# TxCorpi0x/concrete

Measured on AMD Instinct MI355X. Metric: PBS/sec (whole node) at N=1024 batch=4096; achieved HBM GB/s, higher is better.
Workload: dtype u64

## Files before the change

concrete_amd/csrc/pbs.hip:

```cpp
#include <type_traits>

#include "common.hpp"
#include "fft512.hpp"
#include "kernel_util.hpp"
#include "pbs.hpp"
#include "pbs1024_plan.hpp"
#include "pbs_hex.hpp"

namespace chip {

constexpr uint64_t MAGIC_ALL = RND_MAGIC_BITS + (RND_MAGIC_BITS << 22) + (RND_MAGIC_BITS << 43);
constexpr int limb_shift(int li) { return li * 21 + (li > 0 ? 1 : 0); }

#ifndef FWD_LAST_VIA_WINDOW
#define FWD_LAST_VIA_WINDOW 1
#endif
#ifndef FWD_TW2_EARLY
#define FWD_TW2_EARLY 1
#endif
#ifndef DIAG_NOMAC
#define DIAG_NOMAC 0
#endif

#ifndef FWD_XBATCH
#define FWD_XBATCH 2
#endif
#ifndef PAIR_FLAGS
#define PAIR_FLAGS 1
#endif

__device__ __forceinline__ void pair_signal(uint32_t* flags, int w, uint32_t& cnt) {
  asm volatile("" ::: "memory");
  ++cnt;
#if !defined(DIAG_NOXBAR)
  __hip_atomic_store(&flags[w], cnt, __ATOMIC_RELAXED, __HIP_MEMORY_SCOPE_WORKGROUP);
#endif
}
__device__ __forceinline__ void pair_wait(uint32_t* flags, int w, uint32_t cnt, const SyncGuard& guard) {
#if defined(DIAG_NOXBAR)
  (void)flags, (void)w, (void)cnt, (void)guard;
#else
  spin_until_ge(&flags[w ^ 1], cnt, guard);
#endif
  asm volatile("" ::: "memory");
}
__device__ __forceinline__ void xchg_barrier(uint32_t* flags, int w, uint32_t& cnt, const SyncGuard& guard) {
#if defined(DIAG_NOXBAR)
  (void)flags, (void)w, (void)cnt, (void)guard;
  asm volatile("s_waitcnt lgkmcnt(0)" ::: "memory");
#elif PAIR_FLAGS
  asm volatile("s_waitcnt lgkmcnt(0)" ::: "memory");
  ++cnt;
  __hip_atomic_store(&flags[w], cnt, __ATOMIC_RELAXED, __HIP_MEMORY_SCOPE_WORKGROUP);
  spin_until_ge(&flags[w ^ 1], cnt, guard);
#else
  (void)flags, (void)w, (void)cnt, (void)guard;
  pair_barrier();
#endif
}

template <int P, int L, bool RESID, bool STAMPS>
__global__ void __launch_bounds__(P * 128, 2)
pbs1024_pair_kernel(uint64_t* __restrict__ out, const uint64_t* __restrict__ out_idx,
                    const uint64_t* __restrict__ luts, const uint64_t* __restrict__ lut_idx,
                    const uint64_t* __restrict__ in, const uint64_t* __restrict__ in_idx,
                    const cplx* __restrict__ fbsk, uint32_t n, uint32_t base_log, uint32_t num_samples,
                    unsigned long long* __restrict__ resid_out, SyncGuard guard) {
  constexpr int K = 1, K1 = 2, N = 1024, LOG2_2N = 11, LIMBS = 3, RQ = K1 * L;
  constexpr int PER_I = K1 * LIMBS * RQ * 512;
  static_assert(XCH_SLOTS <= (int)PBS1024_XCH_SLOTS, "transpose scratch");
  static_assert(FFT512_TABLE_ENTRIES * sizeof(cplx) == PBS1024_TABLE_BYTES, "table bytes");
  constexpr int NW = 2 * P;
  constexpr int GROUP = L * 512;
  constexpr int NGRP = K1 * K1 * LIMBS;
  constexpr int GLDS = GROUP / 64 / NW;
  static_assert(GROUP % (64 * NW) == 0, "group split");

  extern __shared__ __attribute__((aligned(16))) char smem[];
  cplx* tbl = reinterpret_cast<cplx*>(smem);
  cplx* xch_all = tbl + FFT512_TABLE_ENTRIES;
  cplx* ring = xch_all + NW * PBS1024_XCH_SLOTS;
  uint32_t* pflags = reinterpret_cast<uint32_t*>(ring + 3 * GROUP);

  const int w = __builtin_amdgcn_readfirstlane(threadIdx.x >> 6);
  const int h = w & 1;
  const uint64_t hsign = (uint64_t)h << 63;
  const int lane = threadIdx.x & 63;
  const uint32_t s = blockIdx.x * P + (w >> 1);
  const bool active = s < num_samples;
  cplx* xch = xch_all + w * PBS1024_XCH_SLOTS;
  uint64_t* xch64 = reinterpret_cast<uint64_t*>(xch);
  cplx* mybox = xch;
  const cplx* partnerbox = xch_all + (w ^ 1) * PBS1024_XCH_SLOTS;
  cplx* partnermail = xch_all + (w ^ 1) * PBS1024_XCH_SLOTS;

  static_assert(NGRP % 3 == 0, "ring slot of a group must not depend on the step");
  const cplx* key_w = fbsk + (uint64_t)w * GLDS * 64;
  cplx* ring_w = ring + w * GLDS * 64;
  const uint32_t lane_b = (uint32_t)lane * (uint32_t)sizeof(cplx);
  auto issue_group = [&](const cplx* key_step, int r) __attribute__((always_inline)) {
    const char* src = reinterpret_cast<const char*>(key_step + r * GROUP);
    cplx* dst = ring_w + (r % 3) * GROUP;
#pragma unroll
    for (int j = 0; j < GLDS; ++j)
    {
      const cplx* gp = reinterpret_cast<const cplx*>(src + j * 1024 + lane_b);
      const uint32_t m0 = (uint32_t)(uintptr_t)(lds_ptr_t)(dst + j * 64);
#pragma clang diagnostic push
#pragma clang diagnostic ignored "-Winline-asm"
      asm volatile("s_mov_b32 m0, %1\n\tglobal_load_lds_dwordx4 %0, off" : : "v"(gp), "s"(m0) : "m0", "memory");
#pragma clang diagnostic pop
    }
  };
  if (n > 0) {
    issue_group(key_w, 0);
    issue_group(key_w, 1);
  }

  build_fft512_tables(tbl, threadIdx.x, P * 128);
  if (lane == 0) pflags[w] = 0u;
  uint32_t pcnt = 0;
  __syncthreads();
  const Fft512Tables T = fft512_tables_at(tbl);

  const uint64_t* lwe = in + (active ? (in_idx ? in_idx[s] : s) : 0) * (uint64_t)(n + 1);
  const uint64_t* lut = luts + (active && lut_idx ? lut_idx[s] : 0ull) * (uint64_t)(K1 * N);

  uint64_t B[16];
  {
    const uint32_t bt = active ? modswitch(lwe[n], LOG2_2N) : 0u;
#pragma unroll
    for (int m = 0; m < 16; ++m) {
      const uint32_t src = (uint32_t)(lane + 64 * m + bt) & (2 * N - 1);
      const uint64_t v = active ? lut[h * N + (src & (N - 1))] : 0ull;
      B[m] = src < N ? 0ull - v : v;
    }
  }

  const int nrep = 64 - L * (int)base_log;
  const int logB = (int)base_log;
  const int32_t neg_base = -(1 << logB);
  const uint32_t half_m1 = (1u << (logB - 1)) - 1u;
  double max_resid = 0.0;
  uint64_t acc_t[NSTAMP] = {};
  uint64_t t_begin = 0, tp = 0;
  if constexpr (STAMPS) t_begin = stamp();

  cplx tw3[4];
  fwd_p3_tw(tw3, T, lane);

  uint64_t a_next = active ? lwe[0] : 0ull;
  for (uint32_t i = 0; i < n; ++i) {
    const cplx* key_step = key_w + (uint64_t)i * PER_I;
    const uint64_t ai = a_next;
    if (i + 1 < n) a_next = active ? lwe[i + 1] : 0ull;

    const uint32_t at = modswitch(ai, LOG2_2N);
    if constexpr (STAMPS) {
      tp = stamp();
      acc_t[7] += ai != 0ull && at != 0u;
    }

    uint32_t st[16];
    {
#pragma unroll
      for (int m = 0; m < 16; ++m) xch64[lane + 64 * m] = B[m];
      wave_lds_fence();
      const uint32_t o0 = ((uint32_t)(lane - (int)at) << 3) + 8u * N;
      const uint32_t khi = 1u << (nrep - 33);
      uint64_t rv[16];
#pragma unroll
      for (int m = 0; m < 16; ++m)
        rv[m] = *reinterpret_cast<const uint64_t*>(reinterpret_cast<const char*>(xch64) + ((o0 + 512u * m) & 8191u));
      __builtin_amdgcn_sched_barrier(0);
#pragma unroll
      for (int m = 0; m < 16; ++m) {
        const uint32_t o = o0 + 512u * m;
        const uint32_t s32 = (uint32_t)((int32_t)(o << 18) >> 31);
        const uint64_t rvs = rv[m] ^ (((uint64_t)s32 << 32) | s32);
        const uint64_t x = B[m] + rvs + (uint64_t)(s32 & 1u);
        st[m] = ((uint32_t)(x >> 32) + khi) >> (nrep - 32);
      }
      wave_lds_fence();
    }
    if constexpr (STAMPS) {
      uint64_t t = stamp();
      acc_t[0] += t - tp;
      tp = t;
    }

    cplx Xo[L][4], Xp[L][4];
    constexpr int XB = FWD_XBATCH;
#pragma unroll
    for (int q0 = 0; q0 < L; q0 += XB) {
      const int nq = (q0 + XB <= L) ? XB : L - q0;
      cplx out[XB][4];
      {
#pragma unroll
        for (int t = 0; t < XB; ++t) {
          if (t < nq) {
            cplx v[8];
            int32_t d[16];
#pragma unroll
            for (int m = 0; m < 16; ++m)
              d[m] = decomp_level32(st[m], (uint32_t)((q0 + t) * logB), logB, half_m1, neg_base, q0 + t + 1 < L);
#pragma unroll
            for (int m = 0; m < 8; ++m) v[m] = {(double)d[m], (double)d[m + 8]};
            cplx tw2[4];
            fwd_p2_tw(tw2, T, lane >> 3);
            if (FWD_TW2_EARLY) __builtin_amdgcn_sched_barrier(0);
            fft512_fwd_tw(v, xch, lane, tw2, tw3, hsign, [&]() __attribute__((always_inline)) {
              if (q0 > 0 && t == 0) pair_wait(pflags, w, pcnt, guard);
            });
#pragma unroll
            for (int j = 0; j < 4; ++j) {
              Xo[q0 + t][j] = v[j];
              out[t][j] = v[4 + j];
            }
          }
        }
#pragma unroll
        for (int t = 0; t < XB; ++t)
          if (t < nq)
#pragma unroll
            for (int j = 0; j < 4; ++j) mybox[(t * 4 + j) * 64 + lane] = out[t][j];
      }
      const bool last_batch = q0 + XB >= L;
      if (!last_batch || !FWD_LAST_VIA_WINDOW) {
        xchg_barrier(pflags, w, pcnt, guard);
#pragma unroll
        for (int t = 0; t < XB; ++t)
          if (t < nq)
#pragma unroll
            for (int j = 0; j < 4; ++j) Xp[q0 + t][j] = partnerbox[(t * 4 + j) * 64 + lane];
      }
#pragma unroll
      for (int t = 0; t < XB; ++t)
        if (t < nq)
#pragma unroll
          for (int j = 0; j < 4; ++j) pin(Xo[q0 + t][j]);
      if (q0 + XB < L) pair_signal(pflags, w, pcnt);
    }
    if constexpr (STAMPS) {
      uint64_t t = stamp();
      acc_t[1] += t - tp;
      tp = t;
    }

    auto recombine = [&](const cplx (&v)[8], auto LIc) __attribute__((always_inline)) {
      constexpr int lr = decltype(LIc)::value;
#pragma unroll
      for (int m = 0; m < 8; ++m) {
        const double tr = RND_MAGIC - v[m].re, ti = RND_MAGIC - v[m].im;
        if constexpr (RESID) {
          max_resid = fmax(max_resid, fabs(v[m].re - (RND_MAGIC - tr)));
          max_resid = fmax(max_resid, fabs(v[m].im - (RND_MAGIC - ti)));
        }
        if constexpr (lr == 0) {
          B[m] += (uint64_t)__double_as_longlong(tr) - MAGIC_ALL;
          B[m + 8] += (uint64_t)__double_as_longlong(ti) - MAGIC_ALL;
        } else {
          B[m] += (uint64_t)__double_as_longlong(tr) << limb_shift(lr);
          B[m + 8] += (uint64_t)__double_as_longlong(ti) << limb_shift(lr);
        }
      }
    };
    static_for<0, LIMBS>([&](auto LI) __attribute__((always_inline)) {
      constexpr int li = decltype(LI)::value;
      cplx Ymine[4];
#pragma unroll
      for (int co = 0; co < K1; ++co) {
        cplx Y[4];
        if constexpr (DIAG_NOMAC) {
#pragma unroll
          for (int j = 0; j < 4; ++j) Y[j] = {0.0, 0.0};
        }
#pragma unroll
        for (int ro = 0; ro < K1; ++ro) {
          const int r = (li * K1 + co) * K1 + ro;
          const bool last_step = i + 1 >= n;
          if constexpr (STAMPS) {
            uint64_t t = stamp();
            acc_t[2] += t - tp;
            tp = t;
          }
          if (r + 1 < NGRP || !last_step) wait_vmcnt<GLDS>();
          else wait_vmcnt<0>();
          if constexpr (STAMPS) {
            uint64_t t = stamp();
            acc_t[8] += t - tp;
            tp = t;
          }
#ifndef DIAG_NOBAR
          pair_barrier();
#endif
          if constexpr (STAMPS) {
            uint64_t t = stamp();
            acc_t[5] += t - tp;
            tp = t;
          }
#ifndef DIAG_NODMA
          if (r + 2 < NGRP) issue_group(key_step, r + 2);
          else if (!last_step) issue_group(key_step + PER_I, r + 2 - NGRP);
#endif
          if constexpr (FWD_LAST_VIA_WINDOW && li == 0) {
            if (co == 0 && ro == 0) {
              constexpr int QL = (L - 1) / FWD_XBATCH * FWD_XBATCH;
#pragma unroll
              for (int q = QL; q < L; ++q)
#pragma unroll
                for (int j = 0; j < 4; ++j) Xp[q][j] = partnerbox[((q - QL) * 4 + j) * 64 + lane];
            }
          }
          const cplx* G = ring + (r % 3) * GROUP + (4 * h) * 64 + lane;
          cplx gv[L][4];
#pragma unroll
          for (int q = 0; q < L; ++q)
#pragma unroll
            for (int j = 0; j < 4; ++j) gv[q][j] = G[(q * 8 + j) * 64];
#pragma unroll
          for (int q = 0; q < (DIAG_NOMAC ? 0 : L); ++q) {
#pragma unroll
            for (int j = 0; j < 4; ++j) {
              const cplx x = ro == 0 ? Xo[q][j] : Xp[q][j];
              if (ro == 0 && q == 0) {
                Y[j].re = __builtin_fma(x.re, gv[q][j].re, -x.im * gv[q][j].im);
                Y[j].im = __builtin_fma(x.re, gv[q][j].im, x.im * gv[q][j].re);
              } else {
                Y[j].re = __builtin_fma(x.re, gv[q][j].re, __builtin_fma(-x.im, gv[q][j].im, Y[j].re));
                Y[j].im = __builtin_fma(x.re, gv[q][j].im, __builtin_fma(x.im, gv[q][j].re, Y[j].im));
              }
            }
          }
#pragma unroll
          for (int j = 0; j < 4; ++j) pin(Y[j]);
        }
        if (co == 0) {
#pragma unroll
          for (int j = 0; j < 4; ++j) Ymine[j] = Y[j];
        } else {
#pragma unroll
          for (int j = 0; j < 4; ++j) partnermail[j * 64 + lane] = Y[j];
        }
      }
      if constexpr (STAMPS) {
        uint64_t t = stamp();
        acc_t[2] += t - tp;
        tp = t;
      }
      xchg_barrier(pflags, w, pcnt, guard);
      cplx vp[8];
#pragma unroll
      for (int j = 0; j < 4; ++j) {
        vp[j] = Ymine[j];
        vp[4 + j] = mybox[j * 64 + lane];
      }
      if constexpr (STAMPS) {
        uint64_t t = stamp();
        acc_t[3] += t - tp;
        tp = t;
      }
      cplx gi2[4];
      inv_p2_stage_tw(gi2, T, lane & 7);
      fft512_inv_tw(vp, xch, T, lane, gi2, hsign);
      recombine(vp, LI);
#pragma unroll
      for (int m = 0; m < 16; ++m) pin(B[m]);
      if constexpr (RESID) pin(max_resid);
      if constexpr (STAMPS) {
        uint64_t t = stamp();
        acc_t[4] += t - tp;
        tp = t;
      }
    });
  }

  if constexpr (STAMPS) {
    acc_t[6] = stamp() - t_begin;
    if (lane == 0 && resid_out) {
      unsigned long long* dst = resid_out + ((uint64_t)blockIdx.x * NW + w) * NSTAMP;
      for (int q = 0; q < NSTAMP; ++q) dst[q] = acc_t[q];
    }
  }

  uint64_t* o = out + (active ? (out_idx ? out_idx[s] : s) : 0) * (uint64_t)(K * N + 1);
  if (!active) {
  } else if (h == 0) {
#pragma unroll
    for (int m = 0; m < 16; ++m) xch64[lane + 64 * m] = B[m];
    wave_lds_fence();
#pragma unroll
    for (int m = 0; m < 16; ++m) {
      const int j = lane + 64 * m;
      const uint64_t v = xch64[(N - j) & (N - 1)];
      o[j] = j == 0 ? 0ull - v : v;
    }
  } else if (lane == 0) {
    o[K * N] = 0ull - B[0];
  }

  if constexpr (RESID && !STAMPS) {
    for (int off = 32; off > 0; off >>= 1) max_resid = fmax(max_resid, __shfl_xor(max_resid, off));
    if (lane == 0 && active && resid_out) atomicMax(resid_out, (unsigned long long)__double_as_longlong(max_resid));
  }
}

template <int P, int L, bool RESID, bool STAMPS>
static int launch_pair_t(const PbsArgs& a) {
  const size_t lds = pbs1024_pair_lds_bytes(L, P);
  if (!pbs1024_exact(1, L, a.base_log)) {
    set_error("pbs: N=1024 l=%d logB=%u is outside the exact range", L, a.base_log);
    return -2;
  }
  auto kern = pbs1024_pair_kernel<P, L, RESID, STAMPS>;
  CHIP_CHECK(hipFuncSetAttribute((const void*)kern, hipFuncAttributeMaxDynamicSharedMemorySize, (int)lds));
  const uint32_t blocks = (a.num_samples + P - 1) / P;
  hipLaunchKernelGGL(kern, dim3(blocks), dim3(P * 128), lds, a.stream, a.out, a.out_idx, a.luts, a.lut_idx,
                     a.in, a.in_idx, reinterpret_cast<const cplx*>(a.fbsk), a.n, a.base_log, a.num_samples, a.resid,
                     a.guard);
  hipError_t e = hipGetLastError();
  if (e != hipSuccess) {
    set_error("pbs launch failed: %s", hipGetErrorString(e));
    return -1;
  }
  return 0;
}

static uint32_t device_cus() {
  static uint32_t cus[64] = {};
  int dev = 0;
  CHIP_CHECK(hipGetDevice(&dev));
  if (dev < 0 || dev >= 64) return 256;
  if (!cus[dev]) {
    int n = 0;
    CHIP_CHECK(hipDeviceGetAttribute(&n, hipDeviceAttributeMultiprocessorCount, dev));
    cus[dev] = n > 0 ? (uint32_t)n : 256u;
  }
  return cus[dev];
}

template <int P, int L>
static int launch_pair_p(const PbsArgs& a) {
  static const bool stamps = getenv("CONCRETE_HIP_PBS_STAMPS") && atoi(getenv("CONCRETE_HIP_PBS_STAMPS"));
  if (stamps) return launch_pair_t<P, L, true, true>(a);
  return a.resid ? launch_pair_t<P, L, true, false>(a) : launch_pair_t<P, L, false, false>(a);
}

static PbsArgs pbs_args_range(const PbsArgs& a, uint32_t start, uint32_t count) {
  PbsArgs r = a;
  r.num_samples = count;
  if (a.in_idx) r.in_idx = a.in_idx + start;
  else r.in = a.in + (uint64_t)start * (a.n + 1);
  if (a.out_idx) r.out_idx = a.out_idx + start;
  else r.out = a.out + (uint64_t)start * (a.k * a.N + 1);
  if (a.lut_idx) r.lut_idx = a.lut_idx + start;
  return r;
}

template <int L>
static int launch_pair(const PbsArgs& a) {
  if (a.num_samples == 0) return 0;
  const char* fe = getenv("CONCRETE_HIP_PBS_PAIRS");
  const int forced = fe ? atoi(fe) : 0;
  const uint32_t cus = device_cus();
  const int P = forced == 1 || forced == 2 || forced == 4 ? forced
                : a.num_samples <= cus ? 1 : a.num_samples <= 2 * cus ? 2 : 4;
  if (L == 3) {
    const char* he = getenv("CONCRETE_HIP_PBS_HEX");
    const int hx = he ? atoi(he) : -1;
    if (hx == 1 || hx == 2) return pbs1024_hex_launch(a, hx);
    if (hx != 0 && !fe && !getenv("CONCRETE_HIP_PBS_QUAD") && !getenv("CONCRETE_HIP_PBS_STAMPS")) {
      const Pbs1024Plan plan = plan_pbs1024(a.num_samples, cus);
      uint32_t start = 0;
      int rc = 0;
      if (plan.pair) {
        rc = launch_pair_p<4, L>(pbs_args_range(a, start, plan.pair));
        start += plan.pair;
      }
      if (rc == 0 && plan.hex2) {
        rc = pbs1024_hex_launch(pbs_args_range(a, start, plan.hex2), 2);
        start += plan.hex2;
      }
      if (rc == 0 && plan.hex1) rc = pbs1024_hex_launch(pbs_args_range(a, start, plan.hex1), 1);
      return rc;
    }
  }
  if (L == 3 && P <= 2 && !getenv("CONCRETE_HIP_PBS_STAMPS")) {
    const char* qe = getenv("CONCRETE_HIP_PBS_QUAD");
    const int q = qe ? atoi(qe) : -1;
    if (q == 1 || q == 2) return pbs1024_quad_launch(a, q);
    if (q != 0 && P == 1) return pbs1024_quad_launch(a, 1);
  }
  if (P == 1) return launch_pair_p<1, L>(a);
  if (P == 2) return launch_pair_p<2, L>(a);
  return launch_pair_p<4, L>(a);
}

int pbs_launch(const PbsArgs& a) {
  const KeyKind kind = key_format(a.k, a.N, a.level).kind;
  if (kind == KeyKind::GENERIC) return pbs_generic_launch(a);
  if (kind == KeyKind::N2048) return pbs2048_launch(a);
  if (kind == KeyKind::K2N1024) return pbs1024k2_launch(a);
  if (kind == KeyKind::SMALL) return pbs_small_launch(a);
  if (kind == KeyKind::N1024 && a.limbs == 3) {
    switch (a.level) {
      case 1: return launch_pair<1>(a);
      case 2: return launch_pair<2>(a);
      case 3: return launch_pair<3>(a);
      default: break;
    }
  }
  set_error("unsupported PBS parameters: N=%u k=%u level=%u limbs=%u", a.N, a.k, a.level, a.limbs);
  return -2;
}

}
```

Baseline: 100,800.

## Add frequency-slot pair PBS kernel with mailbox exchange and make it default

Adds a new N=1024, l=3 PBS kernel in which each of eight waves owns one frequency slot. Forward FFT outputs are exchanged through per-wave LDS mailboxes guarded by counter-based signalling, and key loads are software-prefetched PF steps ahead, including across iterations. The goal is to spread the external-product MAC work across waves and overlap the FFT, key loads and exchange. This costs more LDS, atomic counter spins and extra barriers, and with SLOT_DEFAULT the new kernel replaces the pair path in the planned launch.

After: 107,300 (median of 6 runs). 6.4% higher.

```diff
diff --git a/concrete_amd/csrc/pbs.hip b/concrete_amd/csrc/pbs.hip
--- a/concrete_amd/csrc/pbs.hip
+++ b/concrete_amd/csrc/pbs.hip
@@ -405,6 +405,339 @@
   }
 }
 
+#ifndef SLOT_PF
+#define SLOT_PF 6
+#endif
+#ifndef SLOT_FWD_PAIR
+#define SLOT_FWD_PAIR 1
+#endif
+#ifndef SLOT_Y_EARLY
+#define SLOT_Y_EARLY 1
+#endif
+#ifndef SLOT_QMAJOR
+#define SLOT_QMAJOR 1
+#endif
+#ifndef SLOT_DEFAULT
+#define SLOT_DEFAULT 1
+#endif
+constexpr int SLOT_MBOX = 512;
+constexpr size_t pbs1024_pair_slot_lds_bytes() {
+  return PBS1024_TABLE_BYTES + 2 * (size_t)PBS_PAIRS * (PBS1024_XCH_SLOTS + SLOT_MBOX) * 16 + 16;
+}
+
+__device__ __forceinline__ void slot_signal(uint32_t* ctr, int lane, uint32_t& cnt) {
+  asm volatile("" ::: "memory");
+  ++cnt;
+  if (lane == 0) __hip_atomic_fetch_add(ctr, 1u, __ATOMIC_RELAXED, __HIP_MEMORY_SCOPE_WORKGROUP);
+}
+
+template <bool RESID, bool STAMPS>
+__global__ void __launch_bounds__(PBS_PAIRS * 128, 2)
+pbs1024_pair_slot_kernel(uint64_t* __restrict__ out, const uint64_t* __restrict__ out_idx,
+                         const uint64_t* __restrict__ luts, const uint64_t* __restrict__ lut_idx,
+                         const uint64_t* __restrict__ in, const uint64_t* __restrict__ in_idx,
+                         const cplx* __restrict__ fbsk, uint32_t n, uint32_t base_log, uint32_t num_samples,
+                         unsigned long long* __restrict__ resid_out, SyncGuard guard) {
+  constexpr int K = 1, K1 = 2, N = 1024, LOG2_2N = 11, LIMBS = 3, L = 3, P = PBS_PAIRS, NW = 2 * P;
+  constexpr int GROUP = L * 512;
+  constexpr int PER_I = K1 * K1 * LIMBS * GROUP;
+  constexpr int NKEY = LIMBS * K1 * K1 * L;
+  constexpr int PF = SLOT_PF;
+  constexpr int XS = (int)PBS1024_XCH_SLOTS, MB = SLOT_MBOX;
+  static_assert(NW == 8, "one frequency slot per wave");
+  static_assert(NKEY % PF == 0, "a key value's register must not depend on the step");
+  static_assert(XCH_SLOTS <= XS, "transpose scratch");
+
+  extern __shared__ __attribute__((aligned(16))) char smem[];
+  cplx* tbl = reinterpret_cast<cplx*>(smem);
+  cplx* xch_all = tbl + FFT512_TABLE_ENTRIES;
+  cplx* mbox_all = xch_all + NW * XS;
+  uint32_t* ctr = reinterpret_cast<uint32_t*>(mbox_all + NW * MB);
+
+  const int w = __builtin_amdgcn_readfirstlane(threadIdx.x >> 6);
+  const int h = w & 1;
+  const int lane = threadIdx.x & 63;
+  const uint32_t s = blockIdx.x * P + (w >> 1);
+  const bool active = s < num_samples;
+  cplx* xch = xch_all + w * XS;
+  uint64_t* xch64 = reinterpret_cast<uint64_t*>(xch);
+  cplx* mybox = mbox_all + w * MB + lane;
+  cplx* slotbox = mbox_all + w * 64 + lane;
+
+  const bool flip = w >= 4;
+  const cplx* key_w = fbsk + (w * 64 + (flip ? 3 * GROUP : 0));
+  const int gstride = flip ? -GROUP : GROUP;
+  auto key_load = [&](const cplx* key_step, int t) __attribute__((always_inline)) {
+    const int li = t / (K1 * K1 * L), co = t / (K1 * L) % K1, e = t % (K1 * L);
+    const int ro = SLOT_QMAJOR ? e % K1 : e / L, q = SLOT_QMAJOR ? e / K1 : e % L, cr = co * K1 + ro;
+    return (key_step + (li * K1 * K1 * GROUP + q * 512) + cr * gstride)[lane];
+  };
+  cplx g[PF] = {};
+  if (n > 0) {
+#pragma unroll
+    for (int t = 0; t < PF; ++t) g[t] = key_load(key_w, t);
+  }
+
+  build_fft512_tables(tbl, threadIdx.x, P * 128);
+  if (threadIdx.x == 0) *ctr = 0u;
+  uint32_t rcnt = 0;
+  __syncthreads();
+  const Fft512Tables T = fft512_tables_at(tbl);
+
+  const uint64_t* lwe = in + (active ? (in_idx ? in_idx[s] : s) : 0) * (uint64_t)(n + 1);
+  const uint64_t* lut = luts + (active && lut_idx ? lut_idx[s] : 0ull) * (uint64_t)(K1 * N);
+
+  uint64_t B[16];
+  {
+    const uint32_t bt = active ? modswitch(lwe[n], LOG2_2N) : 0u;
+#pragma unroll
+    for (int m = 0; m < 16; ++m) {
+      const uint32_t src = (uint32_t)(lane + 64 * m + bt) & (2 * N - 1);
+      const uint64_t v = active ? lut[h * N + (src & (N - 1))] : 0ull;
+      B[m] = src < N ? 0ull - v : v;
+    }
+  }
+
+  const int nrep = 64 - L * (int)base_log;
+  const int logB = (int)base_log;
+  const int32_t neg_base = -(1 << logB);
+  const uint32_t half_m1 = (1u << (logB - 1)) - 1u;
+  double max_resid = 0.0;
+  uint64_t acc_t[NSTAMP] = {};
+  uint64_t t_begin = 0, tp = 0;
+  auto lap = [&](int k) __attribute__((always_inline)) {
+    if constexpr (STAMPS) {
+      const uint64_t t = stamp();
+      acc_t[k] += t - tp;
+      tp = t;
+    }
+  };
+  if constexpr (STAMPS) t_begin = stamp();
+
+  cplx tw3[4];
+  fwd_p3_tw(tw3, T, lane);
+
+  uint64_t a_next = active && n > 0 ? lwe[0] : 0ull;
+  for (uint32_t i = 0; i < n; ++i) {
+    const cplx* key_step = key_w + (uint64_t)i * PER_I;
+    const cplx* key_next = i + 1 < n ? key_step + PER_I : key_step;
+    const uint64_t ai = a_next;
+    if (i + 1 < n) a_next = active ? lwe[i + 1] : 0ull;
+    const uint32_t at = modswitch(ai, LOG2_2N);
+    if constexpr (STAMPS) {
+      tp = stamp();
+      acc_t[7] += ai != 0ull && at != 0u;
+    }
+
+    uint32_t st[16];
+    {
+#pragma unroll
+      for (int m = 0; m < 16; ++m) xch64[lane + 64 * m] = B[m];
+      wave_lds_fence();
+      const uint32_t o0 = ((uint32_t)(lane - (int)at) << 3) + 8u * N;
+      const uint32_t khi = 1u << (nrep - 33);
+      uint64_t rv[16];
+#pragma unroll
+      for (int m = 0; m < 16; ++m)
+        rv[m] = *reinterpret_cast<const uint64_t*>(reinterpret_cast<const char*>(xch64) + ((o0 + 512u * m) & 8191u));
+      __builtin_amdgcn_sched_barrier(0);
+#pragma unroll
+      for (int m = 0; m < 16; ++m) {
+        const uint32_t o = o0 + 512u * m;
+        const uint32_t s32 = (uint32_t)((int32_t)(o << 18) >> 31);
+        const uint64_t rvs = rv[m] ^ (((uint64_t)s32 << 32) | s32);
+        const uint64_t x = B[m] + rvs + (uint64_t)(s32 & 1u);
+        st[m] = ((uint32_t)(x >> 32) + khi) >> (nrep - 32);
+      }
+      wave_lds_fence();
+    }
+    lap(0);
+
+    cplx X[L][NW];
+    cplx hold[8];
+    (void)hold;
+#pragma unroll
+    for (int q = 0; q < L; ++q) {
+      cplx v[8];
+      int32_t d[16];
+#pragma unroll
+      for (int m = 0; m < 16; ++m)
+        d[m] = decomp_level32(st[m], (uint32_t)(q * logB), logB, half_m1, neg_base, q + 1 < L);
+#pragma unroll
+      for (int m = 0; m < 8; ++m) v[m] = {(double)d[m], (double)d[m + 8]};
+      cplx tw2[4];
+      fwd_p2_tw(tw2, T, lane >> 3);
+      if (FWD_TW2_EARLY) __builtin_amdgcn_sched_barrier(0);
+#if SLOT_FWD_PAIR
+      fft512_fwd_tw(v, xch, lane, tw2, tw3, 0ull, [&]() __attribute__((always_inline)) {
+        if (q == 2) spin_until_ge(ctr, NW * rcnt, guard);
+      });
+      if (q == 0) {
+#pragma unroll
+        for (int k = 0; k < 8; ++k) hold[k] = v[k];
+      } else {
+#pragma unroll
+        for (int k = 0; k < 8; ++k) {
+          if (q == 1) mybox[k * 64] = hold[k], xch[k * 64 + lane] = v[k];
+          else mybox[k * 64] = v[k];
+        }
+        lap(1);
+        pair_barrier();
+        lap(5);
+#pragma unroll
+        for (int u = 0; u < NW; ++u) {
+          if (q == 1) X[0][u] = slotbox[u * MB], X[1][u] = xch_all[u * XS + w * 64 + lane];
+          else X[2][u] = slotbox[u * MB];
+        }
+        slot_signal(ctr, lane, rcnt);
+      }
+#else
+      fft512_fwd_tw(v, xch, lane, tw2, tw3, 0ull, []() __attribute__((always_inline)) {});
+      if (q > 0) spin_until_ge(ctr, NW * rcnt, guard);
+#pragma unroll
+      for (int k = 0; k < 8; ++k) mybox[k * 64] = v[k];
+      lap(1);
+      pair_barrier();
+      lap(5);
+#pragma unroll
+      for (int u = 0; u < NW; ++u) X[q][u] = slotbox[u * MB];
+      slot_signal(ctr, lane, rcnt);
+#endif
+    }
+    lap(1);
+
+    auto recombine = [&](const cplx (&v)[8], auto LIc) __attribute__((always_inline)) {
+      constexpr int lr = decltype(LIc)::value;
+#pragma unroll
+      for (int m = 0; m < 8; ++m) {
+        const double tr = RND_MAGIC - v[m].re, ti = RND_MAGIC - v[m].im;
+        if constexpr (RESID) {
+          max_resid = fmax(max_resid, fabs(v[m].re - (RND_MAGIC - tr)));
+          max_resid = fmax(max_resid, fabs(v[m].im - (RND_MAGIC - ti)));
+        }
+        if constexpr (lr == 0) {
+          B[m] += (uint64_t)__double_as_longlong(tr) - MAGIC_ALL;
+          B[m + 8] += (uint64_t)__double_as_longlong(ti) - MAGIC_ALL;
+        } else {
+          B[m] += (uint64_t)__double_as_longlong(tr) << limb_shift(lr);
+          B[m + 8] += (uint64_t)__double_as_longlong(ti) << limb_shift(lr);
+        }
+      }
+    };
+    auto window = [&](auto LIc, auto COc) __attribute__((always_inline)) {
+      constexpr int li = decltype(LIc)::value, co = decltype(COc)::value;
+      cplx Y[P];
+#pragma unroll
+      for (int e = 0; e < K1 * L; ++e) {
+        const int ro = SLOT_QMAJOR ? e % K1 : e / L, q = SLOT_QMAJOR ? e / K1 : e % L;
+        const int t = (li * K1 + co) * K1 * L + e;
+        const cplx gv = g[t % PF];
+#pragma unroll
+        for (int c = 0; c < P; ++c) {
+          const cplx x = X[q][2 * c + ro];
+          if (e == 0) {
+            Y[c].re = __builtin_fma(x.re, gv.re, -x.im * gv.im);
+            Y[c].im = __builtin_fma(x.re, gv.im, x.im * gv.re);
+          } else {
+            Y[c].re = __builtin_fma(x.re, gv.re, __builtin_fma(-x.im, gv.im, Y[c].re));
+            Y[c].im = __builtin_fma(x.re, gv.im, __builtin_fma(x.im, gv.re, Y[c].im));
+          }
+        }
+        g[t % PF] = t + PF < NKEY ? key_load(key_step, t + PF) : key_load(key_next, t + PF - NKEY);
+      }
+#pragma unroll
+      for (int c = 0; c < P; ++c) pin(Y[c]);
+      if (co == 0) spin_until_ge(ctr, NW * rcnt, guard);
+#pragma unroll
+      for (int c = 0; c < P; ++c) mbox_all[(2 * c + co) * MB + w * 64 + lane] = Y[c];
+    };
+    if (SLOT_Y_EARLY) window(std::integral_constant<int, 0>{}, std::integral_constant<int, 0>{});
+    static_for<0, LIMBS>([&](auto LI) __attribute__((always_inline)) {
+      constexpr int li = decltype(LI)::value;
+      if (!SLOT_Y_EARLY) window(LI, std::integral_constant<int, 0>{});
+      window(LI, std::integral_constant<int, 1>{});
+      lap(2);
+      pair_barrier();
+      lap(5);
+      cplx vp[8];
+#pragma unroll
+      for (int k = 0; k < 8; ++k) vp[k] = mybox[k * 64];
+      slot_signal(ctr, lane, rcnt);
+      lap(3);
+      if constexpr (SLOT_Y_EARLY && li + 1 < LIMBS) {
+        window(std::integral_constant<int, li + 1>{}, std::integral_constant<int, 0>{});
+        lap(2);
+      }
+      cplx gi2[4];
+      inv_p2_stage_tw(gi2, T, lane & 7);
+      fft512_inv_tw(vp, xch, T, lane, gi2, 0ull);
+      recombine(vp, LI);
+#pragma unroll
+      for (int m = 0; m < 16; ++m) pin(B[m]);
+      if constexpr (RESID) pin(max_resid);
+      lap(4);
+    });
+  }
+
+  if constexpr (STAMPS) {
+    acc_t[6] = stamp() - t_begin;
+    if (lane == 0 && resid_out) {
+      unsigned long long* dst = resid_out + ((uint64_t)blockIdx.x * NW + w) * NSTAMP;
+      for (int q = 0; q < NSTAMP; ++q) dst[q] = acc_t[q];
+    }
+  }
+
+  uint64_t* o = out + (active ? (out_idx ? out_idx[s] : s) : 0) * (uint64_t)(K * N + 1);
+  if (!active) {
+  } else if (h == 0) {
+#pragma unroll
+    for (int m = 0; m < 16; ++m) xch64[lane + 64 * m] = B[m];
+    wave_lds_fence();
+#pragma unroll
+    for (int m = 0; m < 16; ++m) {
+      const int j = lane + 64 * m;
+      const uint64_t v = xch64[(N - j) & (N - 1)];
+      o[j] = j == 0 ? 0ull - v : v;
+    }
+  } else if (lane == 0) {
+    o[K * N] = 0ull - B[0];
+  }
+
+  if constexpr (RESID && !STAMPS) {
+    for (int off = 32; off > 0; off >>= 1) max_resid = fmax(max_resid, __shfl_xor(max_resid, off));
+    if (lane == 0 && active && resid_out) atomicMax(resid_out, (unsigned long long)__double_as_longlong(max_resid));
+  }
+}
+
+template <bool RESID, bool STAMPS>
+static int launch_slot_t(const PbsArgs& a) {
+  constexpr int P = PBS_PAIRS;
+  const size_t lds = pbs1024_pair_slot_lds_bytes();
+  static_assert(pbs1024_pair_slot_lds_bytes() <= 160 * 1024, "LDS of one CU");
+  if (!pbs1024_exact(1, 3, a.base_log)) {
+    set_error("pbs: N=1024 l=3 logB=%u is outside the exact range", a.base_log);
+    return -2;
+  }
+  auto kern = pbs1024_pair_slot_kernel<RESID, STAMPS>;
+  CHIP_CHECK(hipFuncSetAttribute((const void*)kern, hipFuncAttributeMaxDynamicSharedMemorySize, (int)lds));
+  const uint32_t blocks = (a.num_samples + P - 1) / P;
+  hipLaunchKernelGGL(kern, dim3(blocks), dim3(P * 128), lds, a.stream, a.out, a.out_idx, a.luts, a.lut_idx,
+                     a.in, a.in_idx, reinterpret_cast<const cplx*>(a.fbsk), a.n, a.base_log, a.num_samples, a.resid,
+                     a.guard);
+  hipError_t e = hipGetLastError();
+  if (e != hipSuccess) {
+    set_error("pbs launch failed: %s", hipGetErrorString(e));
+    return -1;
+  }
+  return 0;
+}
+
+static int launch_slot(const PbsArgs& a) {
+  static const bool stamps = getenv("CONCRETE_HIP_PBS_STAMPS") && atoi(getenv("CONCRETE_HIP_PBS_STAMPS"));
+  if (stamps) return launch_slot_t<true, true>(a);
+  return a.resid ? launch_slot_t<true, false>(a) : launch_slot_t<false, false>(a);
+}
+
 template <int P, int L, bool RESID, bool STAMPS>
 static int launch_pair_t(const PbsArgs& a) {
   const size_t lds = pbs1024_pair_lds_bytes(L, P);
@@ -466,6 +799,9 @@
   const int P = forced == 1 || forced == 2 || forced == 4 ? forced
                 : a.num_samples <= cus ? 1 : a.num_samples <= 2 * cus ? 2 : 4;
   if (L == 3) {
+    const char* se = getenv("CONCRETE_HIP_PBS_SLOT");
+    const int sl = se ? atoi(se) : -1;
+    if (sl == 1) return launch_slot(a);
     const char* he = getenv("CONCRETE_HIP_PBS_HEX");
     const int hx = he ? atoi(he) : -1;
     if (hx == 1 || hx == 2) return pbs1024_hex_launch(a, hx);
@@ -474,7 +810,8 @@
       uint32_t start = 0;
       int rc = 0;
       if (plan.pair) {
-        rc = launch_pair_p<4, L>(pbs_args_range(a, start, plan.pair));
+        const PbsArgs part = pbs_args_range(a, start, plan.pair);
+        rc = (sl == 0 || !SLOT_DEFAULT) ? launch_pair_p<4, L>(part) : launch_slot(part);
         start += plan.pair;
       }
       if (rc == 0 && plan.hex2) {
```
